# focegueda1998/CALM-ViT-DTE

Hardware: AMD Instinct MI355X
Metric: training images/sec (224^2, bs=256/GPU) (higher is better)
Workload: dtype f32; 1 GPU; CALM-ViT small224 cls, 224x224x3 synthetic, bs=256/GPU, fp32 matmuls, fwd+loss+bwd+clip+AdamW; batch resident in HBM when the timed region starts (the trainer's H2D copy of the batch is excluded); global_batch=256, parallelism=dp1, world=1, backend=none (single process), hipgraph=False

## Files before the change

### calm-vit-dte_amd/csrc/gemm.hip

```cpp
#include <atomic>
#include "gemm_common.h"
#include <stdlib.h>

using namespace calm_gemm_detail;

namespace {

struct ReduceP {
    const float* ws; long ws_slice; int nslices;
    float* C; float* Cg[4]; long c_b0, c_rs;
    int M, N, accumulate;
};
__global__ __launch_bounds__(256) void splitk_reduce(const ReduceP q) {
    const long total = (long)q.M * q.N;
    const float* w = q.ws + (long)blockIdx.y * q.nslices * q.ws_slice;
    float* out = q.Cg[0] ? q.Cg[blockIdx.y] : q.C + blockIdx.y * q.c_b0;
    for (long i = (long)blockIdx.x * 256 + threadIdx.x; i < total; i += (long)gridDim.x * 256) {
        float s0 = 0.f, s1 = 0.f;
        int sl = 0;
        for (; sl + 1 < q.nslices; sl += 2) {
            s0 += w[(long)sl * q.ws_slice + i];
            s1 += w[(long)(sl + 1) * q.ws_slice + i];
        }
        if (sl < q.nslices) s0 += w[(long)sl * q.ws_slice + i];
// ... 146 lines not shown
                const double comb = ns > 1 ? (double)a->M * a->N * 4.0 * ns * (group_split ? batch : 1) / 2.0e12 * 2.0e9 : 0.0;
                const double c = pipe_cost(per * ns, mt, nt, nk, ns > 1, f32) + comb;
                if (c < best) { best = c; best_mt = mt; best_nt = nt; best_split = ns; }
            }
        }
    const int mt = best_mt, nt = best_nt, nsplit = best_split;
    p.tiles_m = (a->M + 64 * mt - 1) / (64 * mt);
    p.tiles_n = (a->N + 32 * nt - 1) / (32 * nt);
    p.kpb = kpb;
    p.kb_total = kpb;
    p.reduce_group = 0;
    p.atomic = nsplit > 1;
    p.slices_per_batch = 0;
    if (p.atomic) {
        p.kb_per_z = (kpb + nsplit - 1) / nsplit;
        const int ns = (kpb + p.kb_per_z - 1) / p.kb_per_z;
        if (group_split) {
            p.slices_per_batch = ns;
            p.nz = ns * batch;
        } else {
            p.nz = ns;
        }
    } else {
        p.kb_per_z = kpb;
        p.nz = batch;
    }
    d.family = f32 ? FAM_PIPE32 : FAM_PIPE;
    d.mt = mt;
    d.nt = nt;
    d.items = (long)p.tiles_m * p.tiles_n * p.nz;
    d.grid = dim3((int)(d.items < 256 ? d.items : 256));
    static const int stagger = [] { const char* e = getenv("CALM_PIPE_STAGGER"); return e ? atoi(e) : 0; }();
    p.stagger = d.items > 256 ? stagger : 0;
    {
        auto m8 = [](int64_t x) { return (x & 7) == 0; };
        const bool u8 = !p.atomic && a->c_type == CALM_ST_BF16 && (!a->aux || a->aux_type == CALM_ST_BF16) &&
                        (!a->residual || (a->r_type == CALM_ST_BF16 && m8(a->r_rs) && m8(a->r_b0) && m8(a->r_b1))) &&
                        m8(a->N) && m8(a->c_rs) && m8(a->c_b0) && m8(a->c_b1);
        p.epi_unit = u8 ? 8 : 4;
    }
    plan_combine(a, p, d, p.nz);
    return 0;
}

double f32_tile_cost(long items, int nk, double rows, int width, int slots, double combine) {
    constexpr double KB_FIXED = 192.0, KB_LATENCY = 1100.0, EPILOGUE = 1500.0;
    const long per_cu = (items + 255) / 256;
    const double resident = (double)(per_cu < slots ? per_cu : slots);
    const double kb = rows * width * BK * 2.0 / 256.0 + KB_FIXED;
    const double mfma = (double)per_cu * nk * kb * (resident + 0.5) / resident;
    const double rounds = (double)((items + 256L * slots - 1) / (256L * slots));
    const double lat = rounds * nk * KB_LATENCY;
    return (mfma > lat ? mfma : lat) + rounds * EPILOGUE + combine / 1000.0;
}

int plan_tiles(const calm_gemm_args* a, GemmP& p, Decomp& d, int dtype, bool vec) {
    const int batch = a->batch0 * a->batch1;
    const int bk = dtype == CALM_F32 ? BK : CK;
    p.kpb = (a->K + bk - 1) / bk;
    const bool trivial_epi = !a->bias && !a->col_scale && !a->residual && !a->C_pre && a->act == CALM_ACT_NONE;

    p.tiles_m = (a->M + BM - 1) / BM;
    const int pad128 = (a->N + 127) / 128 * 128, pad96 = (a->N + 95) / 96 * 96;
    int bn = pad96 < pad128 ? 96 : 128;
    const bool grouped_reduce_unsplit = a->n_group && a->reduce_batch && a->split_k <= 1;
    const bool group_split = a->n_group && !a->reduce_batch && a->split_k == 0 && trivial_epi && a->C_group[0] &&
                             p.tiles_m * ((a->N + bn - 1) / bn) * batch < 256 && p.kpb >= 64;
    const bool k_split = group_split || (a->reduce_batch && !grouped_reduce_unsplit) || a->split_k > 1 ||
                         (a->split_k == 0 && batch == 1 && trivial_epi && p.tiles_m * ((a->N + bn - 1) / bn) < 256 &&
                          p.kpb >= 64);
    if (!k_split) {
        const long cus = 256;
        const long nb = grouped_reduce_unsplit ? 1 : batch;
        const long items96 = (long)p.tiles_m * (pad96 / 96) * nb, items128 = (long)p.tiles_m * (pad128 / 128) * nb;
        const long cost96 = (items96 + cus - 1) / cus * 96, cost128 = (items128 + cus - 1) / cus * 128;
        bn = cost96 < cost128 ? 96 : 128;
    }
    bool wide = false;
    if (dtype == CALM_BF16 && !k_split) {
        const long nb = grouped_reduce_unsplit ? 1 : batch;
        const long rows_w = (long)(a->M + WBM - 1) / WBM * WBM;
        wide = 8 * rows_w <= 9 * (long)a->M &&
               rows_w / WBM * ((a->N + WBN - 1) / WBN) * nb >= CALM_GEMM_WIDE_MIN_TILES;
    }
    wide = wide || (dtype == CALM_BF16 && k_split && !a->reduce_batch && (group_split || batch == 1) &&
                    4 * ((long)(a->M + WBM - 1) / WBM * WBM) <= 5 * (long)a->M);
    if (wide) {
        bn = WBN;
        p.tiles_m = (a->M + WBM - 1) / WBM;
    }
    p.tiles_n = (a->N + bn - 1) / bn;
    const int tiles = p.tiles_m * p.tiles_n;

    const int split_slots = wide ? 256 * 2 : bn == 96 ? 256 * CALM_GEMM_WAVES96 : 256 * CALM_GEMM_WAVES;
    if (k_split && !group_split && !a->reduce_batch && batch != 1) return CALM_E_UNSUPP;
    auto split_count = [&](int ntiles, int slots, int min_kb) {
        int nsplit = 1;
        if (group_split) {
            nsplit = slots / (ntiles * batch);
            const int max_split = (p.kpb + min_kb - 1) / min_kb;
            if (nsplit > max_split) nsplit = max_split;
        } else if (a->reduce_batch && !grouped_reduce_unsplit) {
            nsplit = a->split_k > 1 ? a->split_k : slots / ntiles;
            const int max_split = (batch * p.kpb + 7) / 8;
            if (nsplit > max_split) nsplit = max_split;
            if (a->split_k <= 1 && dtype == CALM_BF16) {
                const int cap = ntiles == 1 ? 128 : 256 / ntiles;
                if (nsplit > cap) nsplit = cap;
            }
        } else if (k_split) {
            nsplit = a->split_k > 1 ? a->split_k : slots / ntiles;
            const int max_split = (p.kpb + min_kb - 1) / min_kb;
            if (nsplit > max_split) nsplit = max_split;
            if (a->split_k <= 1 && dtype == CALM_BF16 && !wide && nsplit > 256 / ntiles) nsplit = 256 / ntiles;
        }
        return nsplit < 1 ? 1 : nsplit;
    };
    auto apply_split = [&](int nsplit) {
        p.atomic = 0;
        p.slices_per_batch = 0;
        if (group_split) {
            p.kb_total = batch * p.kpb;
            if (nsplit > 1) {
                p.atomic = 1;
                p.slices_per_batch = nsplit;
            }
        } else if (grouped_reduce_unsplit) {
            p.kb_total = batch * p.kpb;
        } else if (a->reduce_batch) {
            p.atomic = 1;
            p.kb_total = batch * p.kpb;
        } else if (k_split) {
            p.kb_total = p.kpb;
            p.atomic = nsplit > 1;
        } else {
            p.kb_total = batch * p.kpb;
        }
        if (p.slices_per_batch) {
            p.kb_per_z = (p.kpb + nsplit - 1) / nsplit;
            p.slices_per_batch = (p.kpb + p.kb_per_z - 1) / p.kb_per_z;
        } else if (p.atomic) {
            p.kb_per_z = (p.kb_total + nsplit - 1) / nsplit;
        } else if (grouped_reduce_unsplit) {
            p.kb_per_z = p.kb_total;
        } else {
            p.kb_per_z = p.kpb;
        }
        return p.slices_per_batch ? batch * p.slices_per_batch : (p.kb_total + p.kb_per_z - 1) / p.kb_per_z;
    };
    int nsplit = split_count(tiles, split_slots, 16);
    int gy = apply_split(nsplit);
    int nb64 = 0;
#if CALM_GEMM_F32_TILE64
    const int per_out = p.slices_per_batch ? p.slices_per_batch : gy;
    const bool ws_plan = p.atomic && per_out >= CALM_GEMM_WS_MIN_SLICES && (long)a->M * a->N >= 100000;
    if (dtype == CALM_F32 && (!ws_plan || CALM_GEMM_F32_TILE64 == 2)) {
        const bool auto_split = (group_split || (a->reduce_batch && !grouped_reduce_unsplit) || k_split) && a->split_k <= 1;
        auto cost_of = [&](int tiles_m, int tiles_n, int rows_live, int width, int slots, int y) {
            const long items = (long)tiles_m * tiles_n * y;
            const double comb = p.atomic ? 4.0 * a->M * a->N * y : 0.0;
            return f32_tile_cost(items, p.kb_per_z, (double)rows_live / tiles_m, width, slots, comb);
        };
        const int gran = bn == 128 ? 64 : 32;
        double best = CALM_GEMM_F32_TILE64 == 2 ? 1e300 :
                      cost_of(p.tiles_m, p.tiles_n, (a->M + gran - 1) / gran * gran, bn,
                              bn == 96 ? CALM_GEMM_WAVES96 : CALM_GEMM_WAVES, gy);
        int best_split = nsplit;
        const int tm64 = (a->M + 63) / 64, rows64 = (a->M + 15) / 16 * 16;
        for (int nb = 3; nb <= 8; ++nb) {
            const int tn64 = (a->N + 16 * nb - 1) / (16 * nb);
            const int slots = waves64(nb);
            int cand[3] = {split_count(tm64 * tn64, 256 * slots, 16), 0, 0};
            if (auto_split) {
                cand[1] = split_count(tm64 * tn64, 256 * slots, 4);
                cand[2] = split_count(tm64 * tn64, 2 * 256 * slots, 4);
            }
            for (int ns : cand) {
                if (ns < 1) continue;
                const int y = apply_split(ns);
                const double c = cost_of(tm64, tn64, rows64, 16 * nb, slots, y);
                if (y <= 65535 && c < best) {
                    best = c;
                    nb64 = nb;
                    best_split = ns;
                }
            }
        }
        if (nb64) {
            bn = 16 * nb64;
            p.tiles_m = tm64;
            p.tiles_n = (a->N + bn - 1) / bn;
        }
        nsplit = best_split;
        gy = apply_split(nsplit);
    }
#endif
    if (p.atomic && a->c_type != CALM_ST_F32) return CALM_E_UNSUPP;
    if (p.atomic && !p.slices_per_batch && !trivial_epi) return CALM_E_UNSUPP;
    if (gy > 65535) return CALM_E_UNSUPP;
    d.family = wide ? FAM_BF16_WIDE : dtype == CALM_F32 ? FAM_F32 : FAM_BF16;
    d.bn = bn;
    d.nb64 = nb64;
    d.npass = dtype == CALM_BF16X3 ? 3 : 1;
    d.vec = vec;
    d.items = (long)p.tiles_m * p.tiles_n * gy;
    d.grid = dim3(p.tiles_m * p.tiles_n, gy);
    plan_combine(a, p, d, gy);
    return 0;
}

int plan_fp8(const calm_gemm_args* a, GemmP& p, Decomp& d) {
    if (a->b_type != CALM_ST_FP8_E4M3 || a->a_type < CALM_ST_FP8_E4M3 || !a->a_dq || !a->b_dq) return CALM_E_INVAL;
    if (a->dtype != CALM_BF16 || a->a_cs != 1 || a->b_cs != 1 || a->n_group || a->reduce_batch || a->split_k > 1) return CALM_E_UNSUPP;
    if ((a->K & 15) || (a->a_rs & 15) || (a->b_rs & 15) || (a->a_b0 & 15) || (a->a_b1 & 15) || (a->b_b0 & 15) ||
        (a->b_b1 & 15) || !aligned16(a->A) || !aligned16(a->B))
        return CALM_E_LAYOUT;
    const int batch = a->batch0 * a->batch1;
    if (batch > 65535) return CALM_E_UNSUPP;
    p.dq_a = a->a_dq;
    p.dq_b = a->b_dq;
    p.tiles_m = (a->M + WBM - 1) / WBM;
    p.tiles_n = (a->N + WBN - 1) / WBN;
    d.family = FAM_FP8;
    d.items = p.tiles_m * p.tiles_n * batch;
    d.grid = dim3(p.tiles_m * p.tiles_n, batch);
    return 0;
}

int plan_gemm(const calm_gemm_args* a, GemmP& p, Decomp& d) {
    if (!a || !a->A || !a->B || !a->C) return CALM_E_INVAL;
    if (a->M <= 0 || a->N <= 0 || a->K <= 0 || a->batch0 <= 0 || a->batch1 <= 0) return CALM_E_INVAL;
    if (a->dtype != CALM_F32 && a->dtype != CALM_BF16 && a->dtype != CALM_BF16X3) return CALM_E_UNSUPP;
    for (int t : {a->c_type, a->aux_type, a->r_type})
        if (t != CALM_ST_F32 && t != CALM_ST_BF16) return CALM_E_INVAL;
    for (int t : {a->a_type, a->b_type})
        if (t < CALM_ST_F32 || t > CALM_ST_FP8_E5M2) return CALM_E_INVAL;
    const bool fp8 = a->a_type >= CALM_ST_FP8_E4M3 || a->b_type >= CALM_ST_FP8_E4M3;
    const bool any_bf16_tensor = a->a_type || a->b_type || a->c_type || a->aux_type || a->r_type;
    if (any_bf16_tensor && a->dtype != CALM_BF16) return CALM_E_UNSUPP;
    if (a->a_rs != 1 && a->a_cs != 1) return CALM_E_LAYOUT;
    if (a->b_rs != 1 && a->b_cs != 1) return CALM_E_LAYOUT;
    if (a->a_rs >= (1 << 21) || a->a_cs >= (1 << 21) || a->b_rs >= (1 << 21) || a->b_cs >= (1 << 21)) return CALM_E_UNSUPP;
    if (a->act == CALM_ACT_GELU_BWD && !a->aux) return CALM_E_INVAL;
    if (a->act < 0 || a->act > CALM_ACT_GELU_BWD) return CALM_E_INVAL;
    if (a->n_group < 0 || a->n_group > CALM_GEMM_MAX_GROUP) return CALM_E_INVAL;
    if (a->n_group) {
        if (a->batch0 != a->n_group || a->batch1 != 1) return CALM_E_INVAL;
        if (a->C_pre || a->aux || a->residual || a->inv_scale) return CALM_E_UNSUPP;
        for (int g = 0; g < a->n_group; ++g) {
            if ((a->A_group[0] && !a->A_group[g]) || (a->B_group[0] && !a->B_group[g])) return CALM_E_INVAL;
            if (!a->reduce_batch && a->C_group[0] && !a->C_group[g]) return CALM_E_INVAL;
        }
    }

    p.A = a->A; p.B = a->B; p.C = a->C;
    p.a_type = a->a_type; p.b_type = a->b_type; p.c_type = a->c_type; p.aux_type = a->aux_type; p.r_type = a->r_type;
    p.M = a->M; p.N = a->N; p.K = a->K;
    p.batch1 = a->batch1;
    p.a_rs = a->a_rs; p.a_cs = a->a_cs; p.a_b0 = a->a_b0; p.a_b1 = a->a_b1;
    p.b_rs = a->b_rs; p.b_cs = a->b_cs; p.b_b0 = a->b_b0; p.b_b1 = a->b_b1;
    p.c_rs = a->c_rs; p.c_b0 = a->c_b0; p.c_b1 = a->c_b1;
    p.alpha = a->alpha; p.inv_scale = a->inv_scale; p.bias = a->bias; p.col_scale = a->col_scale;
    p.residual = a->residual; p.r_rs = a->r_rs; p.r_b0 = a->r_b0; p.r_b1 = a->r_b1;
    p.C_pre = a->C_pre; p.aux = a->aux;
    p.act = a->act; p.accumulate = a->accumulate;
    p.n_group = a->n_group;
    p.reduce_group = a->n_group && a->reduce_batch;
    for (int g = 0; g < a->n_group; ++g) {
        p.Ag[g] = a->A_group[g];
        p.Bg[g] = a->B_group[g];
        p.Cg[g] = a->C_group[g];
        p.Sg[g] = a->inv_scale_group[g];
    }
    {
        auto m4 = [](int64_t x) { return (x & 3) == 0; };
        bool ev = m4(a->N) && m4(a->c_rs) && m4(a->c_b0) && m4(a->c_b1) && aligned16(a->C) &&
                  (!a->C_pre || aligned16(a->C_pre)) && (!a->aux || aligned16(a->aux)) &&
                  (!a->bias || aligned16(a->bias)) && (!a->col_scale || aligned16(a->col_scale)) &&
                  (!a->residual || (aligned16(a->residual) && m4(a->r_rs) && m4(a->r_b0) && m4(a->r_b1)));
        for (int g = 0; g < a->n_group; ++g) ev = ev && (!a->C_group[g] || aligned16(a->C_group[g]));
        p.epi_vec = ev && CALM_GEMM_VEC_EPILOGUE;
    }
    if (fp8) return plan_fp8(a, p, d);

    const bool akc = a->a_cs == 1, bkc = a->b_cs == 1;
    const int64_t ea = a->a_type == CALM_ST_BF16 ? 7 : 3, eb = a->b_type == CALM_ST_BF16 ? 7 : 3;
    auto mult = [](int64_t x, int64_t mask) { return (x & mask) == 0; };
    bool vec = aligned16(a->A) && aligned16(a->B) && mult(a->a_b0, ea) && mult(a->a_b1, ea) && mult(a->b_b0, eb) &&
               mult(a->b_b1, eb);
    for (int g = 0; g < a->n_group; ++g) vec = vec && aligned16(a->A_group[g]) && aligned16(a->B_group[g]);
    vec = vec && (akc ? (mult(a->K, ea) && mult(a->a_rs, ea)) : (mult(a->M, ea) && mult(a->a_cs, ea)));
    vec = vec && (bkc ? (mult(a->K, eb) && mult(a->b_rs, eb)) : (mult(a->N, eb) && mult(a->b_cs, eb)));
    if (!vec && any_bf16_tensor) return CALM_E_LAYOUT;
    const int dtype = vec ? a->dtype : CALM_F32;
    if (dtype == CALM_BF16 && a->a_type == CALM_ST_BF16 && a->b_type == CALM_ST_BF16 && pipe_enabled()) {
        const int rc = plan_pipe(a, p, d, false);
        if (rc != PIPE_DECLINED) return rc;
    }
    if (vec && a->dtype == CALM_F32 && !any_bf16_tensor && (pipe32_mode() == 1 || (pipe32_mode() == 2 && akc && bkc))) {
        const int rc = plan_pipe(a, p, d, true);
        if (rc != PIPE_DECLINED) return rc;
    }
    return plan_tiles(a, p, d, dtype, vec);
}

calm_gemm_plan to_plan(const GemmP& p, const Decomp& d, bool use_ws) {
    calm_gemm_plan r{d.family, 0, 0, 0, p.tiles_m, p.tiles_n, d.slices_per_out, (int32_t)d.items,
                     (int32_t)(d.grid.x * d.grid.y), 0, use_ws ? 1 : 0, 0};
    switch (d.family) {
    case FAM_F32:       r.tile_m = d.nb64 ? 64 : BM; r.tile_n = d.bn; r.tile_k = BK; r.threads = NTHREADS; break;
    case FAM_BF16:      r.tile_m = BM;  r.tile_n = d.bn; r.tile_k = CK; r.threads = NTHREADS; break;
    case FAM_BF16_WIDE: r.tile_m = WBM; r.tile_n = WBN;  r.tile_k = CK; r.threads = WTHREADS; break;
    case FAM_FP8:       r.tile_m = WBM; r.tile_n = WBN;  r.tile_k = 64; r.threads = WTHREADS; break;
    default:
        r.tile_m = 64 * d.mt; r.tile_n = 32 * d.nt; r.tile_k = d.family == FAM_PIPE32 ? 32 : 64; r.threads = 512;
        r.epi_unit = p.epi_unit;
    }
    return r;
}

int launch_main(const GemmP& p, const Decomp& d, hipStream_t s) {
    const bool akc = p.a_cs == 1, bkc = p.b_cs == 1;
    switch (d.family) {
// ... 71 lines not shown
```

### calm-vit-dte_amd/csrc/gemm_common.h

```cpp
#pragma once
#include "common.h"
#include <type_traits>

namespace calm_gemm_detail {

#ifndef CALM_GEMM_BK
#define CALM_GEMM_BK 16
#endif
constexpr int BM = 128, BK = CALM_GEMM_BK, NTHREADS = 256;
constexpr int CK = 32;
constexpr int WTHREADS = 512, WBM = 256, WBN = 128;
#ifndef CALM_GEMM_WAVES
#define CALM_GEMM_WAVES 4
#endif
#ifndef CALM_GEMM_WAVES96
#define CALM_GEMM_WAVES96 5
#endif
#ifndef CALM_GEMM_F32_TILE64
#define CALM_GEMM_F32_TILE64 1
#endif
#ifndef CALM_GEMM_WAVES64
#define CALM_GEMM_WAVES64 6
#endif
constexpr int waves64(int nb) { return nb == 8 ? 5 : CALM_GEMM_WAVES64; }
#ifndef CALM_GEMM_VEC_EPILOGUE
#define CALM_GEMM_VEC_EPILOGUE 1
#endif
#ifndef CALM_GEMM_KC_SWIZZLE
#define CALM_GEMM_KC_SWIZZLE 1
#endif
#ifndef CALM_GEMM_BF16_DEEP
#define CALM_GEMM_BF16_DEEP 1
#endif
#ifndef CALM_GEMM_BF16_WAVES
#define CALM_GEMM_BF16_WAVES 3
#endif
#ifndef CALM_GEMM_WIDE_MIN_TILES
#define CALM_GEMM_WIDE_MIN_TILES 512
#endif

struct GemmP {
    const void* A; const void* B; void* C;
    int M, N, K;
    int batch1;
    long a_rs, a_cs, a_b0, a_b1;
    long b_rs, b_cs, b_b0, b_b1;
    long c_rs, c_b0, c_b1;
    float alpha;
    const float* inv_scale; const float* bias; const float* col_scale;
    const void* residual; long r_rs, r_b0, r_b1;
    void* C_pre; const void* aux;
    int act, accumulate;
    int kpb;
    int kb_total;
    int kb_per_z;
    int atomic;
    int tiles_m, tiles_n;
    int slices_per_batch;
    int n_group, reduce_group;
    const void* Ag[4]; const void* Bg[4]; void* Cg[4]; const float* Sg[4];
    float* ws; long ws_slice;
    int a_type, b_type, c_type, aux_type, r_type;
    const float* dq_a; const float* dq_b;
    int epi_vec;
    int nz;
    int stagger;
    int epi_unit;
};

template <typename T = float>
__device__ __forceinline__ const T* operand_base(const void* base, const void* const (&tab)[4], int n_group,
                                                 long s0, long s1, int b0, int b1) {
    if (n_group && tab[0]) return reinterpret_cast<const T*>(tab[b0]) + b1 * s1;
    return reinterpret_cast<const T*>(base) + b0 * s0 + b1 * s1;
}
template <bool TYPED>
__device__ __forceinline__ float ld_elem(const void* base, long i, int type) {
    if (TYPED && type == CALM_ST_BF16) return (float)reinterpret_cast<const __bf16*>(base)[i];
    return reinterpret_cast<const float*>(base)[i];
}
template <bool TYPED>
__device__ __forceinline__ void st_elem(void* base, long i, float v, int type) {
    if (TYPED && type == CALM_ST_BF16) reinterpret_cast<__bf16*>(base)[i] = (__bf16)v;
    else reinterpret_cast<float*>(base)[i] = v;
}
typedef __attribute__((address_space(3))) float lds_float;
typedef __attribute__((address_space(3))) f32x4 lds_f32x4;
template <bool TYPED>
__device__ __forceinline__ f32x4 ld_elem4(const void* base, long i, int type) {
    if (TYPED && type == CALM_ST_BF16) {
        typedef __bf16 bf16x4_t __attribute__((ext_vector_type(4)));
        const bf16x4_t b = *reinterpret_cast<const bf16x4_t*>(reinterpret_cast<const __bf16*>(base) + i);
        return f32x4{(float)b[0], (float)b[1], (float)b[2], (float)b[3]};
    }
    return *reinterpret_cast<const f32x4*>(reinterpret_cast<const float*>(base) + i);
}
template <bool TYPED>
__device__ __forceinline__ void st_elem4(void* base, long i, const f32x4& v, int type) {
    if (TYPED && type == CALM_ST_BF16) {
        typedef __bf16 bf16x4_t __attribute__((ext_vector_type(4)));
        *reinterpret_cast<bf16x4_t*>(reinterpret_cast<__bf16*>(base) + i) =
            bf16x4_t{(__bf16)v[0], (__bf16)v[1], (__bf16)v[2], (__bf16)v[3]};
    } else {
        *reinterpret_cast<f32x4*>(reinterpret_cast<float*>(base) + i) = v;
    }
}
__device__ __forceinline__ float group_sigma(const GemmP& p, int g) { return p.Sg[g] ? p.Sg[g][0] : 1.f; }

template <int MT, int NT>
__device__ __forceinline__ void group_rescale(const GemmP& p, f32x16 (&acc)[MT][NT], int g) {
    const float ratio = group_sigma(p, g) / group_sigma(p, g - 1);
#pragma unroll
    for (int i = 0; i < MT; ++i)
#pragma unroll
        for (int j = 0; j < NT; ++j) acc[i][j] *= ratio;
}

template <int IDX, int MT, int NT, class F>
__device__ __forceinline__ void for_each_subtile(F&& f, f32x16 (&acc)[MT][NT]) {
    if constexpr (IDX < MT * NT) {
        f(IDX / NT, IDX % NT, acc[IDX / NT][IDX % NT]);
        for_each_subtile<IDX + 1, MT, NT>(f, acc);
    }
}

template <int MT, int NT, bool TYPED = false>
__device__ __forceinline__ void gemm_epilogue(const GemmP& p, f32x16 (&acc)[MT][NT], int m0, int n0, int wm, int wn,
                                              int r, int h, int z, int sgroup, lds_float* __restrict__ scratch) {
#ifdef CALM_GEMM_NO_EPILOGUE
    if (p.alpha != 12345.f) return;
#endif
    float scale = p.alpha;
    if (p.inv_scale) scale = scale / p.inv_scale[0];
    if (TYPED && p.dq_a) scale *= p.dq_a[0] * p.dq_b[0];
    const int zc = (p.atomic && !p.slices_per_batch) ? 0 : z;
    const int cb0 = zc / p.batch1, cb1 = zc - cb0 * p.batch1;
    const long coff = cb0 * p.c_b0 + cb1 * p.c_b1;
    const int csz = (TYPED && p.c_type == CALM_ST_BF16) ? 2 : 4;
    char* __restrict__ Cb = reinterpret_cast<char*>(p.C) + coff * csz;
    if (p.n_group) {
        scale = scale / group_sigma(p, p.reduce_group ? sgroup : cb0);
        if (!p.reduce_group && p.Cg[0]) Cb = reinterpret_cast<char*>(p.Cg[cb0]) + cb1 * p.c_b1 * csz;
    }
    char* __restrict__ Pb = p.C_pre ? reinterpret_cast<char*>(p.C_pre) + coff * csz : nullptr;
    const char* __restrict__ Xb =
        p.aux ? reinterpret_cast<const char*>(p.aux) + coff * ((TYPED && p.aux_type == CALM_ST_BF16) ? 2 : 4) : nullptr;
    const char* __restrict__ Rb = p.residual ? reinterpret_cast<const char*>(p.residual) +
                                                   (cb0 * p.r_b0 + cb1 * p.r_b1) * ((TYPED && p.r_type == CALM_ST_BF16) ? 2 : 4)
                                             : nullptr;

    const int pM = p.M, pN = p.N, p_act = p.act, p_accumulate = p.accumulate, p_atomic = p.atomic;
    const int c_type = p.c_type, aux_type = p.aux_type, r_type = p.r_type;
    const long c_rs = p.c_rs, r_rs = p.r_rs, ws_slice = p.ws_slice;
    const float* __restrict__ p_bias = p.bias;
    const float* __restrict__ p_col_scale = p.col_scale;
    float* __restrict__ p_ws = p.ws;
    if (p.epi_vec && !p_atomic) {
        const int lane = r + 32 * h, rl = lane >> 3, c4 = 4 * (lane & 7);
        for_each_subtile<0, MT, NT>([&](int i, int j, const f32x16& a) __attribute__((always_inline)) {
            const int col0 = n0 + wn * (32 * NT) + 32 * j, row0 = m0 + wm * (32 * MT) + 32 * i;
            if (col0 >= pN || row0 >= pM) return;
#pragma unroll
            for (int e = 0; e < 16; ++e) scratch[(4 * h + (e & 3) + 8 * (e >> 2)) * 32 + r] = a[e];
            __builtin_amdgcn_fence(__ATOMIC_RELEASE, "wavefront");
            __builtin_amdgcn_wave_barrier();
            __builtin_amdgcn_fence(__ATOMIC_ACQUIRE, "wavefront");
            const int col = col0 + c4;
            const bool col_ok = col < pN;
            const int colc = col_ok ? col : col0;
            const f32x4 bj = p_bias ? *reinterpret_cast<const f32x4*>(p_bias + colc) : f32x4{0.f, 0.f, 0.f, 0.f};
            const f32x4 sj = p_col_scale ? *reinterpret_cast<const f32x4*>(p_col_scale + colc) : f32x4{1.f, 1.f, 1.f, 1.f};
#pragma unroll
            for (int q0 = 0; q0 < 4; q0 += 2) {
                f32x4 v[2], t[2];
                int ro[2];
                bool ok[2];
#pragma unroll
// ... 138 lines not shown
```

### calm-vit-dte_amd/csrc/gemm_f32.hip

```cpp
#include "gemm_common.h"

namespace calm_gemm_detail {

constexpr int LDT = 132;
constexpr int NREG = BK / 2;

template <bool KC, int ROWS, int RP = 128>
struct OperandCursor {
    static constexpr int NR = RP * BK / NTHREADS;
    static constexpr int TPR = RP / 4;
    const float* base;
    unsigned off[NR / 4];
    long step;
    __device__ __forceinline__ void init(const float* origin, long rs, long cs, int row0, int nrows_all, int k0) {
        const int tid = threadIdx.x;
        const int last = min(nrows_all - row0, ROWS) - 1;
        if constexpr (KC) {
            constexpr int KQ = BK / 4, RPP = NTHREADS / KQ;
            base = origin + (long)row0 * rs + k0;
#pragma unroll
            for (int i = 0; i < NR / 4; ++i)
                off[i] = (unsigned)(min((tid / KQ) + RPP * i, last) * rs + 4 * (tid % KQ)) * 4u;
            step = BK;
        } else {
// ... 144 lines not shown
    constexpr int NT = BN_ / (WN * 32);
    constexpr int LDB = BN_ == 128 ? LDT : 100;
    __shared__ __attribute__((aligned(16))) float As[2][BK][LDT];
    __shared__ __attribute__((aligned(16))) float Bs[2][BK][LDB];

    const int tid = threadIdx.x, lane = tid & 63, wave = __builtin_amdgcn_readfirstlane(tid >> 6);
    const int wm = WN == 2 ? wave >> 1 : wave, wn = WN == 2 ? wave & 1 : 0;
    const int r = lane & 31, h = lane >> 5;

    const int lin = remap_tile(p);
    const int tn = lin % p.tiles_n, tm = lin / p.tiles_n;
    const int m0 = tm * BM, n0 = tn * BN_;
    int z, kb_begin, kb_end;
    slice_range(p, z, kb_begin, kb_end);
    if (kb_begin >= kb_end && p.atomic) return;

    f32x16 acc[MT][NT];
#pragma unroll
    for (int i = 0; i < MT; ++i)
#pragma unroll
        for (int j = 0; j < NT; ++j)
#pragma unroll
            for (int e = 0; e < 16; ++e) acc[i][j][e] = 0.f;

    float ra[NREG], rb[NREG];

    OperandCursor<AKC, BM> ca;
    OperandCursor<BKC, BN_> cb;
    const bool wave_live = m0 + wm * (32 * MT) < p.M;
    auto multiply = [&](int buf) {
        if (!wave_live) return;
#pragma unroll
        for (int s = 0; s < BK / 2; ++s) {
            const int kk = 2 * s + h;
            float af[MT], bf[NT];
#pragma unroll
            for (int i = 0; i < MT; ++i) af[i] = As[buf][kk][wm * (32 * MT) + 32 * i + r];
#pragma unroll
            for (int j = 0; j < NT; ++j) bf[j] = Bs[buf][kk][wn * (32 * NT) + 32 * j + r];
#pragma unroll
            for (int i = 0; i < MT; ++i)
#pragma unroll
                for (int j = 0; j < NT; ++j)
                    acc[i][j] = __builtin_amdgcn_mfma_f32_32x32x2f32(af[i], bf[j], acc[i][j], 0, 0, 0);
        }
    };
    auto stash = [&](int buf) {
        store_operand<AKC, VEC, LDT, BM>(As[buf], ra);
        store_operand<BKC, VEC, LDB, BN_>(Bs[buf], rb);
    };

    auto k_loop = [&](auto full_tag) {
        constexpr bool FULL = decltype(full_tag)::value;
        int cur_b = -1;
        auto fetch = [&](int kb) {
            const int b = p.kb_total == p.kpb ? 0 : kb / p.kpb;
            const int k0 = (kb - b * p.kpb) * BK;
            if constexpr (VEC == 4) {
                if (b != cur_b) {
                    const int b0 = b / p.batch1, b1 = b - b0 * p.batch1;
                    ca.init(operand_base(p.A, p.Ag, p.n_group, p.a_b0, p.a_b1, b0, b1), p.a_rs, p.a_cs, m0, p.M, k0);
                    cb.init(operand_base(p.B, p.Bg, p.n_group, p.b_b0, p.b_b1, b0, b1), p.b_rs, p.b_cs, n0, p.N, k0);
                    cur_b = b;
                }
                ca.template load<FULL>(p.K - k0, ra);
                cb.template load<FULL>(p.K - k0, rb);
            } else {
                const int b0 = b / p.batch1, b1 = b - b0 * p.batch1;
                load_operand<AKC, VEC, BM>(operand_base(p.A, p.Ag, p.n_group, p.a_b0, p.a_b1, b0, b1), p.a_rs, p.a_cs,
                                           m0, p.M, k0, p.K, ra);
                load_operand<BKC, VEC, BN_>(operand_base(p.B, p.Bg, p.n_group, p.b_b0, p.b_b1, b0, b1), p.b_rs,
                                            p.b_cs, n0, p.N, k0, p.K, rb);
            }
        };
        if (kb_begin < kb_end) {
            fetch(kb_begin);
            stash(0);
        }
        __syncthreads();
        auto step = [&](int kb, auto stage_tag) {
            constexpr int ST = decltype(stage_tag)::value;
            const bool more = kb + 1 < kb_end;
            if (p.reduce_group && kb != kb_begin && kb % p.kpb == 0) group_rescale<MT, NT>(p, acc, kb / p.kpb);
            if (more) fetch(kb + 1);
            multiply(ST);
            if (more) stash(ST ^ 1);
            __syncthreads();
        };
        for (int kb = kb_begin; kb < kb_end; kb += 2) {
            step(kb, std::integral_constant<int, 0>{});
            if (kb + 1 < kb_end) step(kb + 1, std::integral_constant<int, 1>{});
        }
    };
    if constexpr (VEC == 4) {
        if (p.K % BK == 0) k_loop(std::true_type{});
        else k_loop(std::false_type{});
    } else {
        k_loop(std::false_type{});
    }

    static_assert(sizeof(As) >= 4096 * (NTHREADS / 64), "the epilogue's per-wave scratch lives in the A stages");
    gemm_epilogue<MT, NT>(p, acc, m0, n0, wm, wn, r, h, z, (kb_end - 1) / p.kpb, (lds_float*)(&As[0][0][0]) + 1024 * wave);
}

template <bool AKC, bool BKC, int VEC>
int launch(const GemmP& p, dim3 grid, int bn, hipStream_t s) {
    if (bn == 128) hipLaunchKernelGGL((gemm_f32_kernel<AKC, BKC, VEC, 128>), grid, dim3(NTHREADS), 0, s, p);
    else hipLaunchKernelGGL((gemm_f32_kernel<AKC, BKC, VEC, 96>), grid, dim3(NTHREADS), 0, s, p);
    CALM_LAUNCH_CHECK();
    return 0;
}

int launch_f32(const GemmP& p, dim3 grid, int bn, bool akc, bool bkc, bool vec, hipStream_t s) {
    if (vec) {
        if (akc && bkc) return launch<true, true, 4>(p, grid, bn, s);
        if (akc && !bkc) return launch<true, false, 4>(p, grid, bn, s);
        if (!akc && bkc) return launch<false, true, 4>(p, grid, bn, s);
        return launch<false, false, 4>(p, grid, bn, s);
    }
    if (akc && bkc) return launch<true, true, 1>(p, grid, bn, s);
    if (akc && !bkc) return launch<true, false, 1>(p, grid, bn, s);
    if (!akc && bkc) return launch<false, true, 1>(p, grid, bn, s);
    return launch<false, false, 1>(p, grid, bn, s);
}

#if CALM_GEMM_F32_TILE64
constexpr int EPI16_LD = 20;
template <int NB>
__device__ __forceinline__ void gemm_epilogue16(const GemmP& p, f32x4 (&acc)[NB], int m0, int n0, int wave, int lane,
                                                int z, int sgroup, lds_float* __restrict__ scratch) {
#ifdef CALM_GEMM_NO_EPILOGUE
    if (p.alpha != 12345.f) return;
#endif
    const int row0 = m0 + 16 * wave;
    if (row0 >= p.M) return;
    float scale = p.alpha;
    if (p.inv_scale) scale = scale / p.inv_scale[0];
    const int zc = (p.atomic && !p.slices_per_batch) ? 0 : z;
    const int cb0 = zc / p.batch1, cb1 = zc - cb0 * p.batch1;
    const long coff = cb0 * p.c_b0 + cb1 * p.c_b1;
    float* __restrict__ Cb = reinterpret_cast<float*>(p.C) + coff;
    if (p.n_group) {
        scale = scale / group_sigma(p, p.reduce_group ? sgroup : cb0);
        if (!p.reduce_group && p.Cg[0]) Cb = reinterpret_cast<float*>(p.Cg[cb0]) + cb1 * p.c_b1;
    }
    float* __restrict__ Pb = p.C_pre ? reinterpret_cast<float*>(p.C_pre) + coff : nullptr;
    const float* __restrict__ Xb = p.aux ? reinterpret_cast<const float*>(p.aux) + coff : nullptr;
    const float* __restrict__ Rb =
        p.residual ? reinterpret_cast<const float*>(p.residual) + (cb0 * p.r_b0 + cb1 * p.r_b1) : nullptr;
    const int pM = p.M, pN = p.N, p_act = p.act, p_accumulate = p.accumulate;
    const long c_rs = p.c_rs, r_rs = p.r_rs;
    const float* __restrict__ p_bias = p.bias;
    const float* __restrict__ p_col_scale = p.col_scale;
    if (p.epi_vec && !p.atomic) {
        const int rl = lane >> 2, c4 = 4 * (lane & 3);
        const int row = row0 + rl;
        const bool row_ok = row < pM;
        const int ro = row_ok ? row : row0;
#pragma unroll
        for (int j = 0; j < NB; ++j) {
            const int col0 = n0 + 16 * j;
            if (col0 >= pN) continue;
#pragma unroll
            for (int e = 0; e < 4; ++e) scratch[(4 * (lane >> 4) + e) * EPI16_LD + (lane & 15)] = acc[j][e];
            __builtin_amdgcn_fence(__ATOMIC_RELEASE, "wavefront");
            __builtin_amdgcn_wave_barrier();
            __builtin_amdgcn_fence(__ATOMIC_ACQUIRE, "wavefront");
            const int col = col0 + c4;
            const bool col_ok = col < pN;
            const int colc = col_ok ? col : col0;
            const bool ok = row_ok && col_ok;
            const long ei = (long)ro * c_rs + colc;
            const f32x4 bj = p_bias ? *reinterpret_cast<const f32x4*>(p_bias + colc) : f32x4{0.f, 0.f, 0.f, 0.f};
            const f32x4 sj = p_col_scale ? *reinterpret_cast<const f32x4*>(p_col_scale + colc) : f32x4{1.f, 1.f, 1.f, 1.f};
            f32x4 v = *(const lds_f32x4*)(scratch + rl * EPI16_LD + c4);
#pragma unroll
            for (int c = 0; c < 4; ++c) v[c] = v[c] * scale + bj[c];
            if (Pb && ok) *reinterpret_cast<f32x4*>(Pb + ei) = v;
            if (p_act == CALM_ACT_GELU) {
#pragma unroll
                for (int c = 0; c < 4; ++c) v[c] = gelu_erf_f(v[c]);
            } else if (p_act == CALM_ACT_GELU_BWD) {
                const f32x4 t = *reinterpret_cast<const f32x4*>(Xb + ei);
#pragma unroll
                for (int c = 0; c < 4; ++c) v[c] *= gelu_erf_grad_f(t[c]);
            }
            v *= sj;
            if (Rb) v += *reinterpret_cast<const f32x4*>(Rb + (long)ro * r_rs + colc);
            if (p_accumulate) v += *reinterpret_cast<const f32x4*>(Cb + ei);
            if (ok) *reinterpret_cast<f32x4*>(Cb + ei) = v;
            __builtin_amdgcn_fence(__ATOMIC_RELEASE, "wavefront");
            __builtin_amdgcn_wave_barrier();
        }
        return;
    }
    const int rq = row0 + 4 * (lane >> 4);
#pragma unroll
    for (int j = 0; j < NB; ++j) {
        const int col = n0 + 16 * j + (lane & 15);
        if (col >= pN) continue;
        if (p.atomic) {
            if (p.ws) {
                float* __restrict__ Wb = p.ws + (long)blockIdx.y * p.ws_slice;
#pragma unroll
                for (int e = 0; e < 4; ++e)
                    if (rq + e < pM) Wb[(long)(rq + e) * pN + col] = acc[j][e] * scale;
            } else {
#pragma unroll
                for (int e = 0; e < 4; ++e)
                    if (rq + e < pM) atomicAdd(Cb + (long)(rq + e) * c_rs + col, acc[j][e] * scale);
            }
            continue;
        }
        const float bj = p_bias ? p_bias[col] : 0.f;
        const float sj = p_col_scale ? p_col_scale[col] : 1.f;
        float v[4], t[4];
        long ci[4], ri[4];
#pragma unroll
        for (int e = 0; e < 4; ++e) {
            const int rowc = rq + e < pM ? rq + e : 0;
            ci[e] = (long)rowc * c_rs + col;
            ri[e] = (long)rowc * r_rs + col;
            v[e] = acc[j][e] * scale + bj;
        }
        if (Pb) {
#pragma unroll
            for (int e = 0; e < 4; ++e)
                if (rq + e < pM) Pb[ci[e]] = v[e];
        }
        if (p_act == CALM_ACT_GELU) {
#pragma unroll
            for (int e = 0; e < 4; ++e) v[e] = gelu_erf_f(v[e]);
        } else if (p_act == CALM_ACT_GELU_BWD) {
#pragma unroll
            for (int e = 0; e < 4; ++e) t[e] = Xb[ci[e]];
#pragma unroll
            for (int e = 0; e < 4; ++e) v[e] *= gelu_erf_grad_f(t[e]);
        }
#pragma unroll
        for (int e = 0; e < 4; ++e) v[e] *= sj;
        if (Rb) {
#pragma unroll
            for (int e = 0; e < 4; ++e) t[e] = Rb[ri[e]];
#pragma unroll
            for (int e = 0; e < 4; ++e) v[e] += t[e];
        }
        if (p_accumulate) {
#pragma unroll
            for (int e = 0; e < 4; ++e) t[e] = Cb[ci[e]];
#pragma unroll
            for (int e = 0; e < 4; ++e) v[e] += t[e];
        }
#pragma unroll
        for (int e = 0; e < 4; ++e)
            if (rq + e < pM) Cb[ci[e]] = v[e];
    }
}

template <bool AKC, bool BKC, int VEC, int NB>
__global__ __launch_bounds__(NTHREADS, waves64(NB)) void gemm_f32_t64_kernel(const GemmP p) {
    constexpr int TM = 64, BN_ = 16 * NB;
    constexpr int RB = BN_ <= 64 ? 64 : 128;
    constexpr int LDA = 80, LDB = (BN_ + 15) / 32 * 32 + 16;
    constexpr int NRA = TM * BK / NTHREADS, NRB = RB * BK / NTHREADS;
    __shared__ __attribute__((aligned(16))) float As[2][BK][LDA];
    __shared__ __attribute__((aligned(16))) float Bs[2][BK][LDB];

    const int tid = threadIdx.x, lane = tid & 63, wave = __builtin_amdgcn_readfirstlane(tid >> 6);
    const int r = lane & 15, g = lane >> 4;

    const int lin = remap_tile(p);
    const int tn = lin % p.tiles_n, tm = lin / p.tiles_n;
    const int m0 = tm * TM, n0 = tn * BN_;
    int z, kb_begin, kb_end;
    slice_range(p, z, kb_begin, kb_end);
    if (kb_begin >= kb_end && p.atomic) return;

    f32x4 acc[NB];
#pragma unroll
    for (int j = 0; j < NB; ++j) acc[j] = f32x4{0.f, 0.f, 0.f, 0.f};

    float ra[NRA], rb[NRB];

    OperandCursor<AKC, TM, TM> ca;
    OperandCursor<BKC, BN_, RB> cb;
    const bool wave_live = m0 + 16 * wave < p.M;
    auto multiply = [&](int buf) {
        if (!wave_live) return;
#pragma unroll
        for (int s = 0; s < BK / 4; ++s) {
            const int kk = 4 * s + g;
            const float af = As[buf][kk][16 * wave + r];
            float bf[NB];
#pragma unroll
            for (int j = 0; j < NB; ++j) bf[j] = Bs[buf][kk][16 * j + r];
#pragma unroll
            for (int j = 0; j < NB; ++j) acc[j] = __builtin_amdgcn_mfma_f32_16x16x4f32(af, bf[j], acc[j], 0, 0, 0);
        }
    };
    auto stash = [&](int buf) {
        store_operand<AKC, VEC, LDA, TM, TM>(As[buf], ra);
        store_operand<BKC, VEC, LDB, BN_, RB>(Bs[buf], rb);
    };

    auto k_loop = [&](auto full_tag) {
        constexpr bool FULL = decltype(full_tag)::value;
        int cur_b = -1;
        auto fetch = [&](int kb) {
            const int b = p.kb_total == p.kpb ? 0 : kb / p.kpb;
            const int k0 = (kb - b * p.kpb) * BK;
            if constexpr (VEC == 4) {
                if (b != cur_b) {
                    const int b0 = b / p.batch1, b1 = b - b0 * p.batch1;
                    ca.init(operand_base(p.A, p.Ag, p.n_group, p.a_b0, p.a_b1, b0, b1), p.a_rs, p.a_cs, m0, p.M, k0);
                    cb.init(operand_base(p.B, p.Bg, p.n_group, p.b_b0, p.b_b1, b0, b1), p.b_rs, p.b_cs, n0, p.N, k0);
                    cur_b = b;
                }
                ca.template load<FULL>(p.K - k0, ra);
                cb.template load<FULL>(p.K - k0, rb);
            } else {
                const int b0 = b / p.batch1, b1 = b - b0 * p.batch1;
                load_operand<AKC, VEC, TM, TM>(operand_base(p.A, p.Ag, p.n_group, p.a_b0, p.a_b1, b0, b1), p.a_rs,
                                               p.a_cs, m0, p.M, k0, p.K, ra);
                load_operand<BKC, VEC, BN_, RB>(operand_base(p.B, p.Bg, p.n_group, p.b_b0, p.b_b1, b0, b1), p.b_rs,
                                                p.b_cs, n0, p.N, k0, p.K, rb);
            }
        };
        if (kb_begin < kb_end) {
            fetch(kb_begin);
            stash(0);
        }
        __syncthreads();
        auto step = [&](int kb, auto stage_tag) {
            constexpr int ST = decltype(stage_tag)::value;
            const bool more = kb + 1 < kb_end;
            if (p.reduce_group && kb != kb_begin && kb % p.kpb == 0) {
                const float ratio = group_sigma(p, kb / p.kpb) / group_sigma(p, kb / p.kpb - 1);
#pragma unroll
                for (int j = 0; j < NB; ++j) acc[j] *= ratio;
            }
            if (more) fetch(kb + 1);
            multiply(ST);
            if (more) stash(ST ^ 1);
            __syncthreads();
        };
        for (int kb = kb_begin; kb < kb_end; kb += 2) {
            step(kb, std::integral_constant<int, 0>{});
            if (kb + 1 < kb_end) step(kb + 1, std::integral_constant<int, 1>{});
        }
    };
    if constexpr (VEC == 4) {
        if (p.K % BK == 0) k_loop(std::true_type{});
        else k_loop(std::false_type{});
    } else {
        k_loop(std::false_type{});
    }

    static_assert(sizeof(As) >= sizeof(float) * 16 * EPI16_LD * (NTHREADS / 64), "the epilogue's scratch lives in the A stages");
    gemm_epilogue16<NB>(p, acc, m0, n0, wave, lane, z, (kb_end - 1) / p.kpb,
                        (lds_float*)(&As[0][0][0]) + 16 * EPI16_LD * wave);
}

template <bool AKC, bool BKC, int VEC>
int launch_t64(const GemmP& p, dim3 grid, int nb, hipStream_t s) {
    switch (nb) {
    case 3: hipLaunchKernelGGL((gemm_f32_t64_kernel<AKC, BKC, VEC, 3>), grid, dim3(NTHREADS), 0, s, p); break;
    case 4: hipLaunchKernelGGL((gemm_f32_t64_kernel<AKC, BKC, VEC, 4>), grid, dim3(NTHREADS), 0, s, p); break;
    case 5: hipLaunchKernelGGL((gemm_f32_t64_kernel<AKC, BKC, VEC, 5>), grid, dim3(NTHREADS), 0, s, p); break;
    case 6: hipLaunchKernelGGL((gemm_f32_t64_kernel<AKC, BKC, VEC, 6>), grid, dim3(NTHREADS), 0, s, p); break;
    case 7: hipLaunchKernelGGL((gemm_f32_t64_kernel<AKC, BKC, VEC, 7>), grid, dim3(NTHREADS), 0, s, p); break;
    case 8: hipLaunchKernelGGL((gemm_f32_t64_kernel<AKC, BKC, VEC, 8>), grid, dim3(NTHREADS), 0, s, p); break;
    default: return CALM_E_INVAL;
    }
    CALM_LAUNCH_CHECK();
    return 0;
}

int launch_f32_t64(const GemmP& p, dim3 grid, int nb, bool akc, bool bkc, bool vec, hipStream_t s) {
    if (vec) {
        if (akc && bkc) return launch_t64<true, true, 4>(p, grid, nb, s);
        if (akc && !bkc) return launch_t64<true, false, 4>(p, grid, nb, s);
        if (!akc && bkc) return launch_t64<false, true, 4>(p, grid, nb, s);
        return launch_t64<false, false, 4>(p, grid, nb, s);
    }
    if (akc && bkc) return launch_t64<true, true, 1>(p, grid, nb, s);
    if (akc && !bkc) return launch_t64<true, false, 1>(p, grid, nb, s);
    if (!akc && bkc) return launch_t64<false, true, 1>(p, grid, nb, s);
    return launch_t64<false, false, 1>(p, grid, nb, s);
}
#else
int launch_f32_t64(const GemmP&, dim3, int, bool, bool, bool, hipStream_t) { return CALM_E_UNSUPP; }
#endif

}
```

Measured before the change: 1923 images/sec.

## Add wide 176-column f32 tile64 variant and workspace-slice epilogue for split-K

```diff
diff --git a/calm-vit-dte_amd/csrc/gemm.hip b/calm-vit-dte_amd/csrc/gemm.hip
--- a/calm-vit-dte_amd/csrc/gemm.hip
+++ b/calm-vit-dte_amd/csrc/gemm.hip
@@ -322,9 +322,7 @@
     int gy = apply_split(nsplit);
     int nb64 = 0;
 #if CALM_GEMM_F32_TILE64
-    const int per_out = p.slices_per_batch ? p.slices_per_batch : gy;
-    const bool ws_plan = p.atomic && per_out >= CALM_GEMM_WS_MIN_SLICES && (long)a->M * a->N >= 100000;
-    if (dtype == CALM_F32 && (!ws_plan || CALM_GEMM_F32_TILE64 == 2)) {
+    if (dtype == CALM_F32) {
         const bool auto_split = (group_split || (a->reduce_batch && !grouped_reduce_unsplit) || k_split) && a->split_k <= 1;
         auto cost_of = [&](int tiles_m, int tiles_n, int rows_live, int width, int slots, int y) {
             const long items = (long)tiles_m * tiles_n * y;
@@ -332,13 +330,18 @@
             return f32_tile_cost(items, p.kb_per_z, (double)rows_live / tiles_m, width, slots, comb);
         };
         const int gran = bn == 128 ? 64 : 32;
-        double best = CALM_GEMM_F32_TILE64 == 2 ? 1e300 :
+        const bool wgrad_split = auto_split && !a->reduce_batch;
+        double best = CALM_GEMM_F32_TILE64 == 2 || wgrad_split ? 1e300 :
                       cost_of(p.tiles_m, p.tiles_n, (a->M + gran - 1) / gran * gran, bn,
                               bn == 96 ? CALM_GEMM_WAVES96 : CALM_GEMM_WAVES, gy);
         int best_split = nsplit;
         const int tm64 = (a->M + 63) / 64, rows64 = (a->M + 15) / 16 * 16;
-        for (int nb = 3; nb <= 8; ++nb) {
+        for (int nb = 3; nb <= 11; ++nb) {
+            if (!t64_width(nb) || (t64_wide(nb) && !vec)) continue;
             const int tn64 = (a->N + 16 * nb - 1) / (16 * nb);
+            if (t64_wide(nb) && CALM_GEMM_F32_TILE64 != 2 &&
+                !(wgrad_split ? tn64 >= 3 : (long)tm64 * tn64 * gy <= 256L * waves64(nb)))
+                continue;
             const int slots = waves64(nb);
             int cand[3] = {split_count(tm64 * tn64, 256 * slots, 16), 0, 0};
             if (auto_split) {
diff --git a/calm-vit-dte_amd/csrc/gemm_common.h b/calm-vit-dte_amd/csrc/gemm_common.h
--- a/calm-vit-dte_amd/csrc/gemm_common.h
+++ b/calm-vit-dte_amd/csrc/gemm_common.h
@@ -22,7 +22,13 @@
 #ifndef CALM_GEMM_WAVES64
 #define CALM_GEMM_WAVES64 6
 #endif
-constexpr int waves64(int nb) { return nb == 8 ? 5 : CALM_GEMM_WAVES64; }
+constexpr bool t64_wide(int nb) { return nb == 11; }
+constexpr int waves64(int nb) { return t64_wide(nb) ? 4 : nb == 8 ? 5 : CALM_GEMM_WAVES64; }
+constexpr int T64_NB_ALL = 0x09f8;
+#ifndef CALM_GEMM_F32_T64_NB_MASK
+#define CALM_GEMM_F32_T64_NB_MASK T64_NB_ALL
+#endif
+constexpr bool t64_width(int nb) { return nb >= 3 && nb <= 11 && ((CALM_GEMM_F32_T64_NB_MASK & T64_NB_ALL) >> nb & 1); }
 #ifndef CALM_GEMM_VEC_EPILOGUE
 #define CALM_GEMM_VEC_EPILOGUE 1
 #endif
diff --git a/calm-vit-dte_amd/csrc/gemm_f32.hip b/calm-vit-dte_amd/csrc/gemm_f32.hip
--- a/calm-vit-dte_amd/csrc/gemm_f32.hip
+++ b/calm-vit-dte_amd/csrc/gemm_f32.hip
@@ -320,6 +320,27 @@
     const long c_rs = p.c_rs, r_rs = p.r_rs;
     const float* __restrict__ p_bias = p.bias;
     const float* __restrict__ p_col_scale = p.col_scale;
+    if (p.atomic && p.ws && (pN & 3) == 0) {
+        float* __restrict__ Wb = p.ws + (long)blockIdx.y * p.ws_slice;
+        const int rl = lane >> 2, c4 = 4 * (lane & 3);
+        const int row = row0 + rl;
+#pragma unroll
+        for (int j = 0; j < NB; ++j) {
+            const int col0 = n0 + 16 * j;
+            if (col0 >= pN) continue;
+#pragma unroll
+            for (int e = 0; e < 4; ++e) scratch[(4 * (lane >> 4) + e) * EPI16_LD + (lane & 15)] = acc[j][e] * scale;
+            __builtin_amdgcn_fence(__ATOMIC_RELEASE, "wavefront");
+            __builtin_amdgcn_wave_barrier();
+            __builtin_amdgcn_fence(__ATOMIC_ACQUIRE, "wavefront");
+            const f32x4 v = *(const lds_f32x4*)(scratch + rl * EPI16_LD + c4);
+            const int col = col0 + c4;
+            if (row < pM && col < pN) *reinterpret_cast<f32x4*>(Wb + (long)row * pN + col) = v;
+            __builtin_amdgcn_fence(__ATOMIC_RELEASE, "wavefront");
+            __builtin_amdgcn_wave_barrier();
+        }
+        return;
+    }
     if (p.epi_vec && !p.atomic) {
         const int rl = lane >> 2, c4 = 4 * (lane & 3);
         const int row = row0 + rl;
@@ -428,8 +449,10 @@
 template <bool AKC, bool BKC, int VEC, int NB>
 __global__ __launch_bounds__(NTHREADS, waves64(NB)) void gemm_f32_t64_kernel(const GemmP p) {
     constexpr int TM = 64, BN_ = 16 * NB;
-    constexpr int RB = BN_ <= 64 ? 64 : 128;
+    constexpr int RB = BN_ <= 64 ? 64 : BN_ <= 128 ? 128 : 256;
     constexpr int LDA = 80, LDB = (BN_ + 15) / 32 * 32 + 16;
+    static_assert(LDA % 32 == 16 && LDB % 32 == 16, "ds_read_b32 fragments: the lane groups of a half-wave 16 banks apart");
+    static_assert(LDA >= TM && LDB >= BN_ && LDB % 4 == 0 && BN_ <= RB, "an image row holds the tile; 16-byte stores stay aligned");
     constexpr int NRA = TM * BK / NTHREADS, NRB = RB * BK / NTHREADS;
     __shared__ __attribute__((aligned(16))) float As[2][BK][LDA];
     __shared__ __attribute__((aligned(16))) float Bs[2][BK][LDB];
@@ -538,6 +561,10 @@
     case 6: hipLaunchKernelGGL((gemm_f32_t64_kernel<AKC, BKC, VEC, 6>), grid, dim3(NTHREADS), 0, s, p); break;
     case 7: hipLaunchKernelGGL((gemm_f32_t64_kernel<AKC, BKC, VEC, 7>), grid, dim3(NTHREADS), 0, s, p); break;
     case 8: hipLaunchKernelGGL((gemm_f32_t64_kernel<AKC, BKC, VEC, 8>), grid, dim3(NTHREADS), 0, s, p); break;
+    case 11:
+        if constexpr (VEC == 4) hipLaunchKernelGGL((gemm_f32_t64_kernel<AKC, BKC, VEC, 11>), grid, dim3(NTHREADS), 0, s, p);
+        else return CALM_E_INVAL;
+        break;
     default: return CALM_E_INVAL;
     }
     CALM_LAUNCH_CHECK();
```

Result: no change. 1936 images/sec (median of 6 runs) (+0.7%).
